# bruniss/multi-task-3d-resencoder-unet

Hardware: AMD Instinct MI355X
Metric: train patches/sec (b,c,z,y,x) ResEncM 1x128^3 (higher is better)
Workload: dtype bf16; 1 GPU; cfg2: ResEncM (6 stages, feats [32, 64, 128, 256, 512, 512], blocks [1, 3, 4, 6, 6, 6]), 1-in, heads ['sheet'], patch 128x128x128, batch 2/GPU, full train step (fwd+loss+bwd+allreduce+clip+AdamW); global_batch=2, parallelism=dp1

## Files before the change

include/rxunet.h:

```cpp
#ifndef RXUNET_H
#define RXUNET_H

#include <stddef.h>
#include <stdint.h>

#ifdef __cplusplus
extern "C" {
#endif

#define RX_OK 0
#define RX_EINVAL (-1)
#define RX_EUNSUPPORTED (-2)
#define RX_ELAUNCH (-3)
#define RX_EWORKSPACE (-4)

typedef enum { RX_F32 = 0, RX_BF16 = 1, RX_F16 = 2 } rx_dtype;
typedef enum { RX_ACT_NONE = 0, RX_ACT_SIGMOID = 1, RX_ACT_SOFTMAX = 2 } rx_head_act;

typedef struct {
  void* ptr;
  int32_t n, z, y, x, c, ld;
  int64_t cs;
} rx_act;

// ... 72 lines not shown
                   const float* gate, const float* mult, float* dadd, float* m12, float* dw1, float* db1, float* dw2,
                   float* db2, void* ws, size_t ws_bytes, void* stream);
int rx_instnorm_gate_act_bwd(rx_dtype dt, const rx_act* g, const rx_act* y, const float* stats, const rx_act* out,
                             float slope, const float* mult, const float* dadd, const float* m12, int keep_x,
                             const rx_act* dy, const rx_act* d_residual, int accumulate_residual, void* stream);

int rx_avgpool_fwd(rx_dtype dt, const rx_act* x, const rx_act* y, const int32_t stride[3], void* stream);
int rx_instnorm_act_pool_fwd(rx_dtype dt, const rx_act* y, const float* stats, const rx_act* residual,
                             const rx_act* out, const rx_act* pooled, const int32_t stride[3], float slope,
                             void* stream);
int rx_avgpool_bwd(rx_dtype dt, const rx_act* dy, const rx_act* dx, const int32_t stride[3], int accumulate,
                   void* stream);

int rx_stem_conv_fwd(rx_dtype dt, const float* x_ncdhw, int n, int cin, int z, int y, int x, const float* w,
                     const float* bias, const rx_act* out, const int32_t kernel[3], void* stream);
int rx_stem_conv_fwd_stats(rx_dtype dt, const float* x_ncdhw, int n, int cin, int z, int y, int x, const float* w,
                           const float* bias, const rx_act* out, const int32_t kernel[3], float eps, float* stats,
                           void* ws, size_t ws_bytes, void* stream);
size_t rx_stem_conv_bwd_weight_workspace(int cin, int cout, int taps);
int rx_stem_conv_bwd_weight(rx_dtype dt, const float* x_ncdhw, int n, int cin, int z, int y, int x,
                            const rx_act* dy, float* dw, const int32_t kernel[3], void* ws, size_t ws_bytes,
                            void* stream);

int rx_head_fwd(rx_dtype dt, const rx_act* x, const float* w, const float* b, int k, float* out_ncdhw,
                int act, void* stream);
size_t rx_head_bwd_workspace(const rx_act* x, int k);
int rx_head_bwd(rx_dtype dt, const float* dout_ncdhw, const rx_act* x, const float* w, int k, const rx_act* dx,
                float* dw, float* db, void* ws, size_t ws_bytes, void* stream);

int rx_instnorm_act_head_fwd(rx_dtype dt, const rx_act* y, const float* stats, const rx_act* out, float slope,
                             const float* head_w, const float* head_b, int k, float* out_ncdhw, int act, void* stream);

int rx_instnorm_act_bwd_head(rx_dtype dt, const float* dout_ncdhw, int k, const float* head_w, const rx_act* y,
                             const float* stats, float slope, const rx_act* dy, float* head_dw, float* head_db, void* ws,
                             size_t ws_bytes, void* stream);

size_t rx_channel_sum_workspace(const rx_act* x);
int rx_channel_sum(rx_dtype dt, const rx_act* x, float* out, void* ws, size_t ws_bytes, void* stream);

size_t rx_loss_workspace(int n, int c, long v);
int rx_bce_dice_loss_fwd(const float* logits, const float* target, int n, int c, long v, float alpha, float beta,
                         float smoothing, float eps, float* loss, float* coef, void* ws, size_t ws_bytes,
                         void* stream);
int rx_bce_dice_loss_bwd(const float* logits, const float* target, int n, int c, long v, float alpha, float beta,
                         float smoothing, const float* coef, const float* grad_loss, float* dlogits, void* stream);
int rx_masked_cosine_loss_fwd(const float* pred, const float* target, int n, int c, long v, float* loss, float* coef,
// ... 87 lines not shown
```

multi-task-3d-resencoder-unet_amd/csrc/rx_elementwise.hip:

```cpp
#include <stdarg.h>

#include <math.h>

#include "rx_common.h"
#include <cstdlib>

static thread_local char g_err[512] = "";
void rx_set_error(const char* fmt, ...) {
  va_list ap;
  va_start(ap, fmt);
  vsnprintf(g_err, sizeof(g_err), fmt, ap);
  va_end(ap);
}
extern "C" const char* rx_last_error(void) { return g_err; }
static thread_local const char* g_last_kernel = "";
static thread_local int g_note_seq_ = 0;
void rx_note_kernel(const char* name) { g_last_kernel = name; ++g_note_seq_; }
int rx_note_seq(void) { return g_note_seq_; }
extern "C" const char* rx_last_conv_kernel(void) { return g_last_kernel; }
extern "C" int rx_abi_version(void) { return 1; }
extern "C" int rx_device_arch_ok(void) {
  int dev = 0;
  if (hipGetDevice(&dev) != hipSuccess) return 0;
  hipDeviceProp_t p;
// ... 1808 lines not shown
  (void)TT;
  for (int i = threadIdx.x; i < 27 * Co; i += 256) {
    int t = i / Co, co = i - t * Co;
    float s = red[0][t][co] + red[1][t][co] + red[2][t][co] + red[3][t][co];
    partial[(((size_t)blockIdx.x * Cin + ci) * 27 + t) * Co + co] = s;
  }
}

__global__ __launch_bounds__(256) void stem_wgrad_finalize(const float* __restrict__ partial, int nch, int Cin, int ky, int kx, int TT, int Co,
                                                           float* __restrict__ dw) {
  const int lane = threadIdx.x & 63;
  const int i = blockIdx.x * 4 + (threadIdx.x >> 6);
  if (i >= Co * Cin * TT) return;
  int co = i / (Cin * TT), r = i - co * (Cin * TT), ci = r / TT, t = r - ci * TT;
  int a = t / (ky * kx), b = (t / kx) % ky, c = t % kx;
  int slot = a * 9 + b * 3 + c;
  double s = 0.0;
  for (int k = lane; k < nch; k += 64) s += (double)partial[(((size_t)k * Cin + ci) * 27 + slot) * Co + co];
  s = wave_sum_d(s);
  if (lane == 0) dw[i] = (float)s;
}

int rx_stem_wgrad_mfma_try(rx_dtype dt, const float* x, int n, int cin, int z, int y, int xx, const rx_act* dy, const int32_t kernel[3],
                           float* partial, int max_blocks, int* nblocks_out, hipStream_t st);
#define RX_STEM_CHUNKS 1024
extern "C" size_t rx_stem_conv_bwd_weight_workspace(int cin, int cout, int taps) {
  (void)taps;
  return (size_t)RX_STEM_CHUNKS * cin * 27 * cout * sizeof(float) + 256;
}

extern "C" int rx_stem_conv_bwd_weight(rx_dtype dt, const float* x_ncdhw, int n, int cin, int z, int y, int x, const rx_act* dy, float* dw,
                                       const int32_t kernel[3], void* ws, size_t ws_bytes, void* stream) {
  RX_RECORD(stream, [=, dy_ = RxActV(dy), kernel_ = RxI3V(kernel)](void* s) { return rx_stem_conv_bwd_weight(dt, x_ncdhw, n, cin, z, y, x, dy_.p(), dw, kernel_.v, ws, ws_bytes, s); });
  int rc;
  if ((rc = check_vec_channels(dy, dt, "rx_stem_conv_bwd_weight(dy)"))) return rc;
  if ((rc = check_kernel13(kernel, "rx_stem_conv_bwd_weight"))) return rc;
  if (!x_ncdhw || !dw || !ws || cin < 1 || cin > 16) RX_FAIL(RX_EUNSUPPORTED, "rx_stem_conv_bwd_weight: 1 <= Cin <= 16");
  const int Co = dy->c;
  if (Co > 64 || Co % 4 || 64 % (Co / 4)) RX_FAIL(RX_EUNSUPPORTED, "rx_stem_conv_bwd_weight: Cout must be 4,8,16,32 or 64 (got %d)", Co);
  if (dy->n != n || dy->z != z || dy->y != y || dy->x != x) RX_FAIL(RX_EINVAL, "rx_stem_conv_bwd_weight: geometry mismatch");
  if (ws_bytes < rx_stem_conv_bwd_weight_workspace(cin, Co, 27)) RX_FAIL(RX_EWORKSPACE, "rx_stem_conv_bwd_weight: workspace too small");
  hipStream_t st0 = (hipStream_t)stream;
  {
    int nb = 0;
    if (rx_stem_wgrad_mfma_try(dt, x_ncdhw, n, cin, z, y, x, dy, kernel, (float*)ws, RX_STEM_CHUNKS, &nb, st0) == 1) {
      const int TT0 = kernel[0] * kernel[1] * kernel[2];
      int tot0 = Co * cin * TT0;
      hipLaunchKernelGGL(stem_wgrad_finalize, dim3((tot0 + 3) / 4), dim3(256), 0, st0, (const float*)ws, nb, cin, kernel[1], kernel[2],
                         TT0, Co, dw);
      RX_CHECK_LAUNCH("rx_stem_conv_bwd_weight(mfma)");
      return RX_OK;
    }
  }
  const long NV = (long)n * z * y * x;
  const int VPB = 256 / (Co / 4);
  long chunk = (NV + RX_STEM_CHUNKS - 1) / RX_STEM_CHUNKS;
  chunk = (chunk + VPB - 1) / VPB * VPB;
  int nch = (int)((NV + chunk - 1) / chunk);
  const int TT = kernel[0] * kernel[1] * kernel[2];
  hipStream_t st = (hipStream_t)stream;
  RX_DISPATCH_DTYPE(dt, T, {
    hipLaunchKernelGGL((stem_wgrad_kernel<T>), dim3(nch, 1, cin), dim3(256), 0, st, x_ncdhw, cin, z, y, x, (const T*)dy->ptr, dy->ld,
                       rx_act_voxels(dy) * dy->ld, Co, kernel[0], kernel[1], kernel[2], n, (int)chunk, (float*)ws);
    int tot = Co * cin * TT;
    hipLaunchKernelGGL(stem_wgrad_finalize, dim3((tot + 3) / 4), dim3(256), 0, st, (const float*)ws, nch, cin, kernel[1], kernel[2], TT, Co,
                       dw);
  });
  RX_CHECK_LAUNCH("rx_stem_conv_bwd_weight");
  return RX_OK;
}

#define RX_PACK_PB 40
#ifndef RX_PACK_THREADS
#define RX_PACK_THREADS 1024
#endif

template <typename T>
__device__ __forceinline__ void pack_tile(const float* __restrict__ w, int A, int B, int TT, unsigned inv_tt, T* __restrict__ same,
                                          int flip_same, T* __restrict__ swp, int flip_swap, const int a0, const int b0) {
  extern __shared__ __attribute__((aligned(16))) unsigned char pack_smem[];
  T* L = reinterpret_cast<T*>(pack_smem);
  const int rowlen = 32 * TT;
  const bool full = a0 + 32 <= A && b0 + 32 <= B && sizeof(T) == 2 && (B & 7) == 0 && (A & 7) == 0;
  if (full && TT > 1 && (rowlen & 3) == 0 && ((size_t)B * TT & 3) == 0) {
    const int q4 = rowlen >> 2;
    for (int q = threadIdx.x; q < 32 * q4; q += RX_PACK_THREADS) {
      const int a = q / q4, c = q - a * q4;
      const f32x4 v = *reinterpret_cast<const f32x4*>(w + ((size_t)(a0 + a) * B + b0) * TT + 4 * c);
#pragma unroll
      for (int j = 0; j < 4; ++j) {
        const unsigned r = 4 * c + j;
// ... 524 lines not shown
```

multi-task-3d-resencoder-unet_amd/csrc/rx_stem_wgrad.hip:

```cpp
#include "rx_common.h"

typedef __attribute__((address_space(3))) s16x4 lds_s16x4_s;

template <typename T>
__device__ inline u32x4 pack8(const float (&f)[8]) {
  T v[8];
#pragma unroll
  for (int j = 0; j < 8; ++j) v[j] = Elem<T>::from_f(f[j]);
  return *reinterpret_cast<u32x4*>(v);
}

template <typename T, int NB>
__global__ __launch_bounds__(256) void stem_wgrad_mfma_kernel(const float* __restrict__ x, int Cin, int N, int Z, int Y, int X,
                                                              const T* __restrict__ dy, int ldy, long sy, int kz, int ky, int kx,
                                                              int tiles_per_block, float* __restrict__ partial) {
  constexpr int TZ = 4, TY = 4, TX = 16, HY = TY + 2, HX = TX + 2, HV = (TZ + 2) * HY * HX;
  constexpr int CO = NB * 32;
  __shared__ __attribute__((aligned(16))) T sG[256 * CO];
  __shared__ float sX[4][HV + 8];
  const int tid = threadIdx.x, lane = tid & 63, wave = tid >> 6;
  const int tz_n = (Z + TZ - 1) / TZ, ty_n = (Y + TY - 1) / TY, tx_n = (X + TX - 1) / TX;
  const int NT = N * tz_n * ty_n * tx_n;
  const int t_begin = blockIdx.x * tiles_per_block, t_end = min(NT, t_begin + tiles_per_block);
  const long V = (long)Z * Y * X;
  const int pz = (kz - 1) / 2, py = (ky - 1) / 2, px = (kx - 1) / 2;

  const int tap = lane & 31, h = lane >> 5;
  const int ta = tap / 9, tb = (tap / 3) % 3, tc = tap % 3;
  const bool tap_ok = tap < 27 && ta < kz && tb < ky && tc < kx;
  const int toff = tap_ok ? ((ta - pz) * HY + (tb - py)) * HX + (tc - px) : 0;
  const int g16 = lane >> 4, half = g16 & 1, ah = g16 >> 1, l15 = lane & 15, q4 = l15 >> 2, p4 = l15 & 3;

  f32x16 acc[4][NB];
#pragma unroll
  for (int c = 0; c < 4; ++c)
#pragma unroll
    for (int a = 0; a < NB; ++a)
#pragma unroll
      for (int r = 0; r < 16; ++r) acc[c][a][r] = 0.f;

  constexpr int GP = CO / 8;
  constexpr int XP = (HV + 255) / 256;
  u32x4 gq[GP];
  float xq[4][XP];
  auto prefetch = [&](int tile) {
    int tx = tile % tx_n, t1 = tile / tx_n;
    int ty = t1 % ty_n, t2 = t1 / ty_n;
    int tz = t2 % tz_n, n = t2 / tz_n;
    const int z0 = tz * TZ, y0 = ty * TY, x0 = tx * TX;
#pragma unroll
    for (int p = 0; p < GP; ++p) {
      const int i = tid + 256 * p;
      const int v = i / (CO / 8), cv = i - v * (CO / 8);
      const int z = z0 + (v >> 6), y = y0 + ((v >> 4) & 3), xx = x0 + (v & 15);
      u32x4 val = u32x4{0u, 0u, 0u, 0u};
      if (z < Z && y < Y && xx < X) val = *reinterpret_cast<const u32x4*>(dy + n * sy + ((long)(z * Y + y) * X + xx) * ldy + cv * 8);
      gq[p] = val;
    }
#pragma unroll
    for (int ci = 0; ci < 4; ++ci) {
      if (ci < Cin) {
        const float* xc = x + ((long)n * Cin + ci) * V;
#pragma unroll
        for (int p = 0; p < XP; ++p) {
          const int i = tid + 256 * p;
          const int hx = i % HX, t = i / HX, hy = t % HY, hz = t / HY;
          const int z = z0 + hz - 1, y = y0 + hy - 1, xx = x0 + hx - 1;
          float v = 0.f;
          if (i < HV && (unsigned)z < (unsigned)Z && (unsigned)y < (unsigned)Y && (unsigned)xx < (unsigned)X) v = xc[((long)z * Y + y) * X + xx];
          xq[ci][p] = v;
        }
      }
    }
  };
  if (t_begin < t_end) prefetch(t_begin);
  for (int tile = t_begin; tile < t_end; ++tile) {
    __syncthreads();
#pragma unroll
    for (int p = 0; p < GP; ++p) {
      const int i = tid + 256 * p;
      const int v = i / (CO / 8), c = (i - v * (CO / 8)) * 8;
      *reinterpret_cast<u32x4*>(sG + ((c >> 5) * 256 + v) * 32 + (c & 31)) = gq[p];
    }
#pragma unroll
    for (int ci = 0; ci < 4; ++ci)
      if (ci < Cin)
#pragma unroll
        for (int p = 0; p < XP; ++p)
          if (tid + 256 * p < HV) sX[ci][tid + 256 * p] = xq[ci][p];
    __syncthreads();
    if (tile + 1 < t_end) prefetch(tile + 1);
#pragma unroll
    for (int kk = 0; kk < 4; ++kk) {
      const int s = wave * 4 + kk;
      const int hrow = (((s >> 2) + 1) * HY + ((s & 3) + 1)) * HX + 1;
      u32x4 af[NB];
#pragma unroll
      for (int a = 0; a < NB; ++a) {
        const T* p0 = sG + (a * 256 + 16 * s + 8 * ah + q4) * 32 + 16 * half + 4 * p4;
        s16x4 t0 = __builtin_amdgcn_ds_read_tr16_b64_v4i16((lds_s16x4_s*)(p0));
        s16x4 t1 = __builtin_amdgcn_ds_read_tr16_b64_v4i16((lds_s16x4_s*)(p0 + 4 * 32));
        u32x2 lo = __builtin_bit_cast(u32x2, t0), hi = __builtin_bit_cast(u32x2, t1);
        af[a] = u32x4{lo[0], lo[1], hi[0], hi[1]};
      }
      for (int ci = 0; ci < Cin; ++ci) {
// ... 13 lines not shown
    }
  }
  __shared__ float red[4][32][33];
  const int col = lane & 31, fh = lane >> 5;
  for (int ci = 0; ci < Cin; ++ci)
    for (int a = 0; a < NB; ++a) {
      __syncthreads();
#pragma unroll
      for (int r = 0; r < 16; ++r) {
        const int row = (r & 3) + 8 * (r >> 2) + 4 * fh;
        float v = ci == 0 ? acc[0][a][r] : ci == 1 ? acc[1][a][r] : ci == 2 ? acc[2][a][r] : acc[3][a][r];
        red[wave][row][col] = v;
      }
      __syncthreads();
      for (int i = tid; i < 27 * 32; i += 256) {
        const int t = i >> 5, co = i & 31;
        float s = red[0][co][t] + red[1][co][t] + red[2][co][t] + red[3][co][t];
        partial[(((size_t)blockIdx.x * Cin + ci) * 27 + t) * CO + a * 32 + co] = s;
      }
    }
}

int rx_stem_wgrad_mfma_try(rx_dtype dt, const float* x, int n, int cin, int z, int y, int xx, const rx_act* dy, const int32_t kernel[3],
                           float* partial, int max_blocks, int* nblocks_out, hipStream_t st) {
  if (dt == RX_F32 || (dy->c != 32 && dy->c != 64) || dy->ld % 8 || ((uintptr_t)dy->ptr & 15) || cin > 4) return 0;
  const int NT = n * ((z + 3) / 4) * ((y + 3) / 4) * ((xx + 15) / 16);
  int blocks = NT < max_blocks ? NT : max_blocks;
  if (blocks > 768) blocks = 768;
  const int per = (NT + blocks - 1) / blocks;
  blocks = (NT + per - 1) / per;
  const long sy = rx_act_voxels(dy) * (long)dy->ld;
#define RX_SW(TT, NBB)                                                                                                           \
  hipLaunchKernelGGL((stem_wgrad_mfma_kernel<TT, NBB>), dim3(blocks), dim3(256), 0, st, x, cin, n, z, y, xx, (const TT*)dy->ptr, \
                     dy->ld, sy, kernel[0], kernel[1], kernel[2], per, partial)
  if (dt == RX_BF16) {
    if (dy->c == 32) RX_SW(bf16_t, 1); else RX_SW(bf16_t, 2);
  } else {
    if (dy->c == 32) RX_SW(f16_t, 1); else RX_SW(f16_t, 2);
  }
#undef RX_SW
  *nblocks_out = blocks;
  return 1;
}


#define RX_STEM_NOTAP 0x40000000
template <typename T, bool STATS = false, int KSM = 7>
__global__ __launch_bounds__(256) void stem_fwd_mfma_kernel(const float* __restrict__ x, int Cin, int N, int Z, int Y, int X,
                                                            const float* __restrict__ w, const float* __restrict__ bias, T* __restrict__ out,
                                                            int ldo, long so, int kz, int ky, int kx, int tiles_per_block,
                                                            int blocks_per_sample = 0, float* __restrict__ stat_part = nullptr) {
  constexpr int TZ = 4, TY = 4, TX = 16, HY = TY + 2, HX = TX + 2, HV = (TZ + 2) * HY * HX;
  constexpr int XP = (HV + 255) / 256;
  __shared__ float sX[4][HV + 8];
  __shared__ int sOff[128];
  const int tid = threadIdx.x, lane = tid & 63, wave = tid >> 6;
  const int TT = kz * ky * kx, K = Cin * TT, KS = (K + 15) / 16;
// ... 155 lines not shown
```

multi-task-3d-resencoder-unet_amd/engine/lib.py:

```python
import ctypes
import os
from ctypes import POINTER, c_char_p, c_double, c_float, c_int, c_int32, c_long, c_size_t, c_void_p

import torch

_HERE = os.path.dirname(os.path.abspath(__file__))
LIB_PATH = os.environ.get("RX_LIBRARY") or os.path.join(os.path.dirname(_HERE), "csrc", "librxunet.so")

RX_F32, RX_BF16, RX_F16 = 0, 1, 2
RX_ACT_NONE, RX_ACT_SIGMOID, RX_ACT_SOFTMAX = 0, 1, 2
DTYPE_CODE = {torch.float32: RX_F32, torch.bfloat16: RX_BF16, torch.float16: RX_F16}
RX_SW_U8, RX_SW_U16, RX_SW_F32 = 0, 1, 2
RX_SW_SCALE, RX_SW_ZSCORE = 0, 1
RX_SW_BLEND_AVERAGE, RX_SW_BLEND_UNIT, RX_SW_BLEND_NONE = 0, 1, 2
RX_SW_CAST_U8, RX_SW_CAST_U16 = 0, 1
RX_AUG_PW_NONE, RX_AUG_PW_AFFINE, RX_AUG_PW_PLANE, RX_AUG_PW_NOISE = 0, 1, 2, 3
RX_AUG_G3_NONE, RX_AUG_G3_FILTER, RX_AUG_G3_DOWNSCALE = 0, 1, 2
RX_AUG_MAX_K, RX_AUG_MAX_BOXES = 21, 4


class RxError(RuntimeError):
    pass


# ... 38 lines not shown
    "rx_instnorm_stats_mask": (c_int, [c_void_p, c_void_p, c_int, c_void_p]),
    "rx_instnorm_fwd": (c_int, [c_int, _P, c_float, c_void_p, _P, _P, c_float, c_void_p, c_size_t, c_void_p]),
    "rx_instnorm_act_bwd": (c_int, [c_int, _P, _P, c_void_p, _P, c_float, _P, _P, c_int, c_void_p, c_size_t,
                                    c_void_p]),
    "rx_instnorm_act_bwd_res": (c_int, [c_int, _P, _P, c_void_p, _P, c_float, _P, I3, _P, _P, c_void_p, c_size_t, c_void_p]),
    "rx_se_workspace": (c_size_t, [_P]),
    "rx_se_gate_fwd": (c_int, [c_int, _P, c_void_p, c_void_p, _PSE, c_void_p, c_void_p, c_void_p, c_void_p, c_void_p, c_size_t,
                               c_void_p]),
    "rx_instnorm_gate_act_fwd": (c_int, [c_int, _P, c_void_p, c_void_p, c_int, _P, _P, c_float, c_void_p]),
    "rx_se_gate_bwd": (c_int, [c_int, _P, _P, c_void_p, _P, c_float, c_void_p, _PSE, c_void_p, c_void_p, c_void_p, c_void_p,
                               c_void_p, c_void_p, c_void_p, c_void_p, c_void_p, c_void_p, c_void_p, c_size_t, c_void_p]),
    "rx_instnorm_gate_act_bwd": (c_int, [c_int, _P, _P, c_void_p, _P, c_float, c_void_p, c_void_p, c_void_p, c_int, _P, _P,
                                         c_int, c_void_p]),
    "rx_avgpool_fwd": (c_int, [c_int, _P, _P, I3, c_void_p]),
    "rx_instnorm_act_pool_fwd": (c_int, [c_int, _P, c_void_p, _P, _P, _P, I3, c_float, c_void_p]),
    "rx_avgpool_bwd": (c_int, [c_int, _P, _P, I3, c_int, c_void_p]),
    "rx_stem_conv_fwd": (c_int, [c_int, c_void_p, c_int, c_int, c_int, c_int, c_int, c_void_p, c_void_p, _P, I3,
                                 c_void_p]),
    "rx_stem_conv_fwd_stats": (c_int, [c_int, c_void_p, c_int, c_int, c_int, c_int, c_int, c_void_p, c_void_p, _P, I3,
                                       c_float, c_void_p, c_void_p, c_size_t, c_void_p]),
    "rx_stem_conv_bwd_weight_workspace": (c_size_t, [c_int, c_int, c_int]),
    "rx_stem_conv_bwd_weight": (c_int, [c_int, c_void_p, c_int, c_int, c_int, c_int, c_int, _P, c_void_p, I3,
                                        c_void_p, c_size_t, c_void_p]),
    "rx_head_fwd": (c_int, [c_int, _P, c_void_p, c_void_p, c_int, c_void_p, c_int, c_void_p]),
    "rx_head_bwd_workspace": (c_size_t, [_P, c_int]),
    "rx_instnorm_act_head_fwd": (c_int, [c_int, _P, c_void_p, _P, c_float, c_void_p, c_void_p, c_int, c_void_p, c_int, c_void_p]),
    "rx_instnorm_act_bwd_head": (c_int, [c_int, c_void_p, c_int, c_void_p, _P, c_void_p, c_float, _P, c_void_p, c_void_p, c_void_p, c_size_t,
                                         c_void_p]),
    "rx_grad_norm_clip_partials": (ctypes.c_long, [c_int, c_void_p]),
    "rx_grad_norm_clip": (c_int, [c_int, c_void_p, c_void_p, c_float, c_void_p, ctypes.c_long, c_void_p, c_void_p]),
    "rx_head_bwd": (c_int, [c_int, c_void_p, _P, c_void_p, c_int, _P, c_void_p, c_void_p, c_void_p, c_size_t,
                            c_void_p]),
    "rx_channel_sum_workspace": (c_size_t, [_P]),
    "rx_channel_sum": (c_int, [c_int, _P, c_void_p, c_void_p, c_size_t, c_void_p]),
    "rx_loss_workspace": (c_size_t, [c_int, c_int, c_long]),
    "rx_bce_dice_loss_fwd": (c_int, [c_void_p, c_void_p, c_int, c_int, c_long, c_float, c_float, c_float, c_float, c_void_p,
                                     c_void_p, c_void_p, c_size_t, c_void_p]),
    "rx_bce_dice_loss_bwd": (c_int, [c_void_p, c_void_p, c_int, c_int, c_long, c_float, c_float, c_float, c_void_p, c_void_p,
                                     c_void_p, c_void_p]),
    "rx_masked_cosine_loss_fwd": (c_int, [c_void_p, c_void_p, c_int, c_int, c_long, c_void_p, c_void_p, c_void_p, c_size_t,
                                          c_void_p]),
    "rx_masked_cosine_loss_bwd": (c_int, [c_void_p, c_void_p, c_int, c_int, c_long, c_void_p, c_void_p, c_void_p, c_void_p]),
    "rx_adamw_pack": (c_int, [c_int, c_void_p, c_void_p, c_void_p, c_void_p, c_void_p, c_double, c_double, c_double, c_double, c_double,
                              c_int, c_int, c_int, c_int, c_int, c_void_p, c_void_p, c_void_p]),
    "rx_adamw_flat_multi": (c_int, [c_int, c_void_p, c_void_p, c_void_p, c_void_p, c_void_p, c_void_p, c_double, c_double, c_double,
                                    c_double, c_double, c_int, c_void_p]),
# ... 80 lines not shown
```

multi-task-3d-resencoder-unet_amd/engine/ops.py:

```python
from ctypes import byref, c_void_p

import numpy as np
import torch

from . import lib as _l
from .lib import I3, RxAct, check, load, stream_ptr

_WS = {}
_PROF = None


def set_profiler(p):
    global _PROF
    _PROF = p


class LaunchProfiler:

    def __init__(self):
        self.pending = []
        self.groups = {}
        self.pending_hbm = []
        self.hbm = {}

# ... 450 lines not shown

def stem_conv_fwd(x_ncdhw, w, bias, out, kernel):
    n, cin, z, y, x = x_ncdhw.shape
    assert x_ncdhw.dtype == torch.float32 and x_ncdhw.is_contiguous()
    check(load().rx_stem_conv_fwd(_code(out.dtype), _ptr(x_ncdhw), n, cin, z, y, x, _ptr(w), _ptr(bias),
                                  byref(out.desc()), I3(*kernel), stream_ptr()), "rx_stem_conv_fwd")


def stem_conv_fwd_stats(x_ncdhw, w, bias, out, kernel, stats, eps=1e-5, ws=None):
    n, cin, z, y, x = x_ncdhw.shape
    assert x_ncdhw.dtype == torch.float32 and x_ncdhw.is_contiguous()
    ws = workspace() if ws is None else ws
    check(load().rx_stem_conv_fwd_stats(_code(out.dtype), _ptr(x_ncdhw), n, cin, z, y, x, _ptr(w), _ptr(bias),
                                        byref(out.desc()), I3(*kernel), float(eps), _ptr(stats), *_ws_args(ws), stream_ptr()),
          "rx_stem_conv_fwd_stats")


def stem_conv_bwd_weight(x_ncdhw, dy, dw, kernel, ws=None):
    n, cin, z, y, x = x_ncdhw.shape
    need = load().rx_stem_conv_bwd_weight_workspace(cin, dy.c, 27)
    ws = workspace(need) if ws is None else ws
    check(load().rx_stem_conv_bwd_weight(_code(dy.dtype), _ptr(x_ncdhw), n, cin, z, y, x, byref(dy.desc()), _ptr(dw),
                                         I3(*kernel), *_ws_args(ws), stream_ptr()), "rx_stem_conv_bwd_weight")


def head_fwd(x, w, b, out_ncdhw, act=_l.RX_ACT_NONE):
    k = w.shape[0]
    check(load().rx_head_fwd(_code(x.dtype), byref(x.desc()), _ptr(w), _ptr(b), k, _ptr(out_ncdhw), int(act),
                             stream_ptr()), "rx_head_fwd")


def head_bwd(dout_ncdhw, x, w, dx, dw, db, ws=None):
    k = w.shape[0]
    need = load().rx_head_bwd_workspace(byref(x.desc()), k)
    ws = workspace(need) if ws is None else ws
    check(load().rx_head_bwd(_code(x.dtype), _ptr(dout_ncdhw), byref(x.desc()), _ptr(w), k,
                             byref(dx.desc()) if dx is not None else None, _ptr(dw), _ptr(db), *_ws_args(ws),
                             stream_ptr()), "rx_head_bwd")


def instnorm_act_head_fwd(y, stats, out, w, b, out_ncdhw, act, slope=0.01):
    check(load().rx_instnorm_act_head_fwd(_code(y.dtype), byref(y.desc()), _ptr(stats), byref(out.desc()) if out is not None else None,
                                          float(slope), _ptr(w), _ptr(b), w.shape[0], _ptr(out_ncdhw), int(act), stream_ptr()),
          "rx_instnorm_act_head_fwd")


# ... 153 lines not shown
se_gate_fwd = _hbm("se_gate_fwd(linesum+gate)", lambda y, *a, **k: _tb(y))(se_gate_fwd)
instnorm_gate_act_fwd = _hbm("in_gate_act_fwd", lambda y, stats, mult, keep_x, out, slope=0.01, residual=None:
                             _tb(y) + _tb(out) + _tb(residual))(instnorm_gate_act_fwd)
se_gate_bwd = _hbm("se_gate_bwd(linesums+gate)", lambda g, y, stats, out, *a, **k: _tb(g) + _tb(y) + _tb(out))(se_gate_bwd)
instnorm_gate_act_bwd = _hbm("in_gate_act_bwd",
                             lambda g, y, stats, out, slope, mult, dadd, m12, keep_x, dy, d_residual=None, accumulate_residual=False:
                             _bwd_bytes(g, y, out, dy, d_residual, accumulate_residual))(instnorm_gate_act_bwd)
avgpool_fwd = _hbm("avgpool_fwd", lambda x, y, stride: _tb(x) + _tb(y))(avgpool_fwd)
instnorm_act_pool_fwd = _hbm("in_act_pool_fwd", lambda y, stats, out, pooled, stride, slope=0.01, residual=None:
                             _tb(y) + _tb(out) + _tb(pooled) + _tb(residual))(instnorm_act_pool_fwd)
avgpool_bwd = _hbm("avgpool_bwd", lambda dy, dx, stride, accumulate=False: _tb(dy) + _tb(dx) * (2 if accumulate else 1))(avgpool_bwd)
head_fwd = _hbm("head_fwd", lambda x, w, b, out_ncdhw, act=0: _tb(x) + out_ncdhw.numel() * 4)(head_fwd)
head_bwd = _hbm("head_bwd", lambda dout_ncdhw, x, w, dx, dw, db, ws=None: dout_ncdhw.numel() * 4 + _tb(x) + _tb(dx))(head_bwd)
instnorm_act_head_fwd = _hbm("in_act_head_fwd", lambda y, stats, out, w, b, out_ncdhw, act, slope=0.01:
                             _tb(y) + _tb(out) + out_ncdhw.numel() * 4)(instnorm_act_head_fwd)
instnorm_act_bwd_head = _hbm("in_act_bwd_head(colreduce+apply)", lambda dout_ncdhw, w, y, stats, dy, slope=0.01, ws=None, dw=None, db=None:
                             dout_ncdhw.numel() * 4 + _tb(y) + _tb(dy))(instnorm_act_bwd_head)
channel_sum = _hbm("channel_sum", lambda x, out, ws=None: _tb(x))(channel_sum)
pack_conv_weight = _hbm("pack", _pack_bytes)(pack_conv_weight)
pack_convT_weight = _hbm("pack", _pack_bytes)(pack_convT_weight)
stem_conv_fwd = _hbm("stem_conv_fwd", lambda x_ncdhw, w, bias, out, kernel: x_ncdhw.numel() * 4 + _tb(out))(stem_conv_fwd)
stem_conv_fwd_stats = _hbm("stem_conv_fwd", lambda x_ncdhw, w, bias, out, kernel, stats, eps=1e-5, ws=None: x_ncdhw.numel() * 4 + _tb(out))(stem_conv_fwd_stats)
stem_conv_bwd_weight = _hbm("stem_conv_bwd_weight", lambda x_ncdhw, dy, dw, kernel, ws=None: x_ncdhw.numel() * 4 + _tb(dy))(stem_conv_bwd_weight)
convT3d_fwd = _hbm("convT_fwd", lambda x, w_fwd, bias, y, stride, ws=None: _tb(x) + _tb(y))(convT3d_fwd)
convT3d_bwd_data = _hbm("convT_bwd_data", lambda dy, w_bwd, dx, stride, accumulate=False, ws=None:
                        _tb(dy) + _tb(dx) * (2 if accumulate else 1))(convT3d_bwd_data)
convT3d_bwd_weight = _hbm("convT_bwd_weight", lambda x, dy, dw, stride, ws=None: _tb(x) + _tb(dy))(convT3d_bwd_weight)
```

multi-task-3d-resencoder-unet_amd/engine/plan.py:

```python
from dataclasses import dataclass, field
from typing import Callable, Dict, List, Optional

import os

import torch
from torch import nn

from . import lib as _l
from . import ops
from .ops import Act


class UnsupportedConfig(NotImplementedError):
    pass


_SIDE_STREAMS: Dict[str, "torch.cuda.Stream"] = {}


def side_stream(device):
    key = str(device)
    st = _SIDE_STREAMS.get(key)
    if st is None:
        st = _SIDE_STREAMS[key] = torch.cuda.Stream(device=device)
# ... 57 lines not shown
        spatial = tuple(in_shape[2:])
        if self.two_d:
            spatial = (1,) + spatial
        self.B, self.Cin, self.spatial = B, Cin, spatial

        self.params: List[nn.Parameter] = []
        self._pidx: Dict[int, int] = {}
        self.packs: List[dict] = []
        self.enc_tape: List[Rec] = []
        self.dec_tapes: List[List[Rec]] = []
        self.fwd: List[Callable] = []
        self.bwd: List[Callable] = []
        self.dy_pool: Dict[tuple, Act] = {}
        self._gbase: Dict[int, torch.Tensor] = {}
        self.outputs: Dict[str, torch.Tensor] = {}
        self.bytes_alloc = 0
        self._x = None
        self._dlogits: Dict[str, torch.Tensor] = {}
        self._grads: List[Optional[torch.Tensor]] = []
        self.grad_order: List[int] = []
        self.grad_sync = None
        import os
        self.overlap_wgrad = os.environ.get("RX_OVERLAP_WGRAD", "1") != "0"
        self.dy_ring = 4
        self._side = None
        self._ws2 = None
        self._dy_turn: Dict[tuple, int] = {}
        self._dy_free: Dict[int, int] = {}
        self._dy_ev: Dict[int, int] = {}
        self._ev_fork = None
        self._ev_join = None
        self._pack_groups = None
        self._gates: List[dict] = []
        self._drops: List[dict] = []
        self._shadows: List[dict] = []
        self._shadow_of: Dict[int, dict] = {}
        self._pad_idx: Dict[int, dict] = {}
        self._pad_done: List[int] = []
        self.use_programs = os.environ.get("RX_PROGRAMS", "1") == "1"
        self._pstate: Dict[tuple, dict] = {}
        self._gflat = None
        self._gviews: Dict[int, torch.Tensor] = {}
        self._marks: List[tuple] = []
        self._recording = None
        self._on_side = False
        self._use_gstore = False
# ... 512 lines not shown
                        f.append(lambda a=a: ops.avgpool_fwd(a["x"].act, a["y"].act, a["stride"]))
                elif rec.kind == "copy":
                    f.append(lambda a=a: ops.avgpool_fwd(a["x"].act, a["y"].act, (1, 1, 1)))
                elif rec.kind == "head":
                    if a.get("fwd_fused"):
                        continue

                    def step(a=a):
                        w2 = a["w"].view(a["k"], -1)
                        ops.head_fwd(a["x"].act, w2, a["b"], a["out"], a["act"] if P._apply_act else _l.RX_ACT_NONE)
                    f.append(step)

    def _dy_for(self, y: AT):
        key = (y.act.dims, y.act.c)
        turn = self._dy_turn.get(key, 0)
        self._dy_turn[key] = (turn + 1) % self.dy_ring
        slot = key + (turn,)
        if slot not in self.dy_pool:
            t = torch.empty((*y.act.dims, y.act.c), dtype=self.dtype, device=self.device)
            self.bytes_alloc += t.numel() * t.element_size()
            self.dy_pool[slot] = Act(t)
        return self.dy_pool[slot]

    def _gen_backward(self):
        P = self
        b = self.bwd
        cat_written = {}

        def mark_cat(cat):
            cat_written[cat.act.key] = True

        def view_written(at):
            return at.written or cat_written.get(at.act.key, False)

        def new_grad(idx):
            sync = P.grad_sync
            ent = P._pad_idx.get(idx)
            if ent is not None:
                if ent["gpad"] is None:
                    ent["gpad"] = torch.empty(tuple(ent["sh"].shape), dtype=torch.float32, device=P.device)
                P._pad_done.append(idx)
                return ent["gpad"]
            if sync is not None:
                g = sync.alloc(idx)
            elif P._use_gstore:
                g = P._gviews[idx]
# ... 60 lines not shown

                    def step(a=a, gx=gx, hinfo=hinfo):
                        dl = P._dlogits.get(a["name"])
                        if dl is None:
                            gx.t.zero_()
                            if P.grad_sync is not None:
                                for i in (a["widx"], a["bidx"]):
                                    new_grad(i).zero_()
                                    done(i)
                            return
                        if hinfo.get("dw_fused"):
                            return
                        dw, db = new_grad(a["widx"]), new_grad(a["bidx"])
                        ops.head_bwd(dl, a["x"].act, a["w"].view(a["k"], -1), None if hinfo["fused"] else gx, dw, db)
                        done(a["widx"])
                        done(a["bidx"])
                    order += [a["widx"], a["bidx"]]
                    b.append(step)
                elif rec.kind == "inact":
                    out, y, res = a["out"], a["y"], a["res"]
                    gout = self._grad_buf(out) if out.gact is None else out.gact
                    if not view_written(out):
                        raise RuntimeError(f"plan bug: gradient of {out.name} is consumed before it is produced")
                    dy = self._dy_for(y)
                    y.gact = dy
                    gres, acc = None, False
                    if res is not None and res.needs_grad:
                        gres = self._grad_buf(res)
                        acc = view_written(res)
                        res.written = True
                        wrote(res, "gres")
                    gw = getattr(out, "_gw", (None, None))
                    if (gw[0] == "head" and a["gate"] is None and res is None and self.dtype != torch.float32
                            and out.act.voxels > 512):
                        heads = [r.a for r in tape if r.kind == "head" and r.a["x"] is out]
                        if len(heads) == 1 and heads[0]["k"] <= 4:
                            a["head_src"] = heads[0]
                            gw[1]["fused"] = True
                            if heads[0].get("fwd_fused") and heads[0]["w"] is self.params[heads[0]["widx"]]:
                                a["head_dw_fused"] = True
                                gw[1]["dw_fused"] = True
                    if (gw[0] == "conv" and a["gate"] is None and res is None and self.dtype != torch.float32
                            and out.act.full_buffer and out.act.root is None and out.act.c % 32 == 0 and out.act.voxels > 512
                            and out.act.dims[3] >= 16):
                        a["m12"] = torch.empty((self.B, out.act.c, 2), dtype=torch.float32, device=self.device)
                        a["m12_valid"] = False
                        gw[1]["inact"] = a
                    def gistep(a=a, gout=gout, dy=dy, gres=gres, acc=acc):
                        g = a["gate"]
                        before_dy_write(dy)
                        if g["se"] is None and g.get("scale_now") is None:
                            ops.instnorm_act_bwd(gout, a["y"].act, a["stats"],
                                                 a["out"].act if (a["slope"] != 1.0 and a["res"] is not None) else None, dy,
                                                 a["slope"], gres, acc)
                            return
                        grads = [new_grad(i) for i in g["se"]["idx"]] if g["se"] is not None else [None] * 4
                        ops.se_gate_bwd(gout, a["y"].act, a["stats"], a["out"].act, a["slope"], P._se_args(g), g["pooled"],
                                        g["hidden"], g["gate"], g["mult"], g["dadd"], g["m12"], *grads,
                                        path_scale=g.get("scale_now"))
                        ops.instnorm_gate_act_bwd(gout, a["y"].act, a["stats"], a["out"].act, a["slope"], g["mult"], g["dadd"],
                                                  g["m12"], g["keep_x"], dy, gres, acc)
                        if g["se"] is not None:
                            for i in g["se"]["idx"]:
                                done(i)
                    if a["gate"] is not None:
                        if a["gate"]["se"] is not None:
                            order += a["gate"]["se"]["idx"]
                        b.append(gistep)
                        continue

                    pend = getattr(out, "_pool_pending", None)
                    out._pool_pending = None
                    fuse_res = gres is not None and not acc and res is not None and y.act.voxels > 512
                    if pend is not None and not fuse_res:
                        b.append(lambda pend=pend: ops.avgpool_bwd(pend["gy"], pend["gx"], pend["stride"], True))
                        pend = None
                    if fuse_res:
                        def rstep(a=a, gout=gout, dy=dy, gres=gres, pend=pend):
                            before_dy_write(dy)
                            ops.instnorm_act_bwd_res(gout, a["y"].act, a["stats"], a["out"].act, dy, gres, a["slope"],
                                                     pool_dy=pend["gy"] if pend is not None else None,
                                                     pool_stride=pend["stride"] if pend is not None else (1, 1, 1))
                        b.append(rstep)
                        continue

                    def istep(a=a, gout=gout, dy=dy, gres=gres, acc=acc):
                        before_dy_write(dy)
                        mask_out = a["out"].act if (a["slope"] != 1.0 and a["res"] is not None) else None
                        hs = a.get("head_src")
                        dl = P._dlogits.get(hs["name"]) if hs is not None else None
                        if dl is not None and a.get("head_dw_fused"):
                            dw, db = new_grad(hs["widx"]), new_grad(hs["bidx"])
                            ops.instnorm_act_bwd_head(dl, hs["w"].view(hs["k"], -1), a["y"].act, a["stats"], dy, a["slope"],
                                                      dw=dw.view(hs["k"], -1), db=db)
                            done(hs["widx"])
                            done(hs["bidx"])
                        elif dl is not None:
                            ops.instnorm_act_bwd_head(dl, hs["w"].view(hs["k"], -1), a["y"].act, a["stats"], dy, a["slope"])
                        elif a.get("m12_valid"):
                            a["m12_valid"] = False
                            ops.instnorm_act_bwd_apply(gout, a["y"].act, a["stats"], mask_out, dy, a["m12"], a["slope"], gres, acc)
                        elif "inbwd_reduce" in skip and a["y"].act.voxels > 512:
                            if "m12x" not in a:
                                a["m12x"] = torch.zeros((self.B, a["y"].act.c, 2), dtype=torch.float32, device=self.device)
                            ops.instnorm_act_bwd_apply(gout, a["y"].act, a["stats"], mask_out, dy, a["m12x"], a["slope"], gres, acc)
                        else:
                            ops.instnorm_act_bwd(gout, a["y"].act, a["stats"], mask_out, dy, a["slope"], gres, acc)
                    b.append(istep)
                elif rec.kind in ("conv", "stem"):
                    y = a["y"]
                    dy = y.gact

                    def wstep(a=a, dy=dy, kind=rec.kind):
                        dw = new_grad(a["widx"])
                        db = new_grad(a["bidx"]) if a["bidx"] is not None else None

                        def launches(ws):
                            if "wgrad" in skip and kind != "stem":
                                pass
                            elif kind == "stem":
                                ops.stem_conv_bwd_weight(P._x, dy, dw, a["kernel"], ws)
                            else:
                                ops.conv3d_bwd_weight(a["x"].act, dy, dw, a["kernel"], a["stride"], ws)
                            done(a["widx"])
                            if db is not None:
                                ops.channel_sum(dy, db, ws)
                                done(a["bidx"])
                        side_run(launches, dy)
                    order += [a["widx"]] + ([a["bidx"]] if a["bidx"] is not None else [])
                    b.append(wstep)
                    if rec.kind == "conv" and a["x"].needs_grad:
                        x = a["x"]
                        gx = self._grad_buf(x)
                        acc = view_written(x)
                        x.written = True
                        if x.act.full_buffer:
                            mark_cat(x)
# ... 439 lines not shown
            if g is None:
                continue
            g = g.detach()
            if g.dtype != torch.float32 or not g.is_contiguous():
                g = g.float().contiguous()
            if graphs or programs:
                buf = self._dl_static.get(k)
                if buf is None or buf.shape != g.shape:
                    buf = self._dl_static[k] = torch.empty_like(g)
                buf.copy_(g)
                g = buf
            self._dlogits[k] = g.unsqueeze(2) if self.two_d else g
        self._ensure_side()
        self.net._weights_epoch = getattr(self.net, "_weights_epoch", 0) + 1
        self._grads = [None] * len(self.params)
        if programs:
            sync = self.grad_sync
            self._use_gstore = sync is None
            if sync is None:
                self._grad_store()
            else:
                sync.persistent = True
                sync.begin(self)
            key = ("b", tuple(sorted(self._dlogits)), id(sync) if sync is not None else 0, self.overlap_wgrad)
            st, replayed = self._programmed(key, self._backward_body,
                                            segments=self._replay_backward_segments if sync is not None else None)
            if replayed:
                self._pad_done = [idx for idx in set(self.grad_order) if idx in self._pad_idx]
            if replayed and sync is None:
                for idx in set(self.grad_order):
                    self._grads[idx] = self._gviews[idx]
            grads = self._backward_finish()
            return [t.detach() if t is not None else None for t in grads]
        self._use_gstore = False
        if self.grad_sync is not None:
            self.grad_sync.persistent = False
            self.grad_sync.begin(self)
        if not graphs:
            self._backward_body()
            return self._backward_finish()
        key = ("b", tuple(sorted(self._dlogits)))
        st = self._gstate.get(key)
        if st is not None and st.get("graph") is not None:
            owned = st["owned"]
            for p in self.params:
                gr = p.grad
                if gr is not None and gr.data_ptr() in owned:
                    p.grad = gr.clone()

        def body():
            self._backward_body()
            return self._backward_finish()
        st = self._graphed(key, body)
        grads = st["result"]
        if st["eager"]:
            return grads
        if "owned" not in st:
            st["owned"] = {t.data_ptr() for t in grads if t is not None}
        return [t.detach() if t is not None else None for t in grads]
```

Before: 119.4 patches/s.

## Fuse instnorm-activation backward into stem conv weight-gradient kernel

Adds an INACT variant of the stem MFMA wgrad kernel. It recomputes the instance-norm plus leaky-ReLU backward (dy from g, y, stats, m12) on the fly while staging tiles into shared memory. The planner detects the stem conv followed by an instnorm whose residual needs no gradient, and skips materialising the full-resolution stem dy tensor and the separate wgrad read of it. In exchange the kernel does extra loads of y and per-channel stats. There is also a fallback path that allocates a dy buffer lazily when fusion is not applicable.

Result: no change. 119.7 patches/s, median of 4 (+0.3%).

```diff
diff --git a/include/rxunet.h b/include/rxunet.h
--- a/include/rxunet.h
+++ b/include/rxunet.h
@@ -118,6 +118,10 @@
                             const rx_act* dy, float* dw, const int32_t kernel[3], void* ws, size_t ws_bytes,
                             void* stream);
 
+int rx_stem_conv_bwd_weight_inact(rx_dtype dt, const float* x_ncdhw, int n, int cin, int z, int y, int x, const rx_act* g,
+                                  const rx_act* in_y, const float* in_stats, const float* m12, float slope, float* dw,
+                                  const int32_t kernel[3], int* fused, void* ws, size_t ws_bytes, void* stream);
+
 int rx_head_fwd(rx_dtype dt, const rx_act* x, const float* w, const float* b, int k, float* out_ncdhw,
                 int act, void* stream);
 size_t rx_head_bwd_workspace(const rx_act* x, int k);
diff --git a/multi-task-3d-resencoder-unet_amd/csrc/rx_elementwise.hip b/multi-task-3d-resencoder-unet_amd/csrc/rx_elementwise.hip
--- a/multi-task-3d-resencoder-unet_amd/csrc/rx_elementwise.hip
+++ b/multi-task-3d-resencoder-unet_amd/csrc/rx_elementwise.hip
@@ -1854,7 +1854,8 @@
 }
 
 int rx_stem_wgrad_mfma_try(rx_dtype dt, const float* x, int n, int cin, int z, int y, int xx, const rx_act* dy, const int32_t kernel[3],
-                           float* partial, int max_blocks, int* nblocks_out, hipStream_t st);
+                           float* partial, int max_blocks, int* nblocks_out, hipStream_t st, const rx_act* in_y,
+                           const float* in_stats, const float* m12, float slope);
 #define RX_STEM_CHUNKS 1024
 extern "C" size_t rx_stem_conv_bwd_weight_workspace(int cin, int cout, int taps) {
   (void)taps;
@@ -1875,7 +1876,8 @@
   hipStream_t st0 = (hipStream_t)stream;
   {
     int nb = 0;
-    if (rx_stem_wgrad_mfma_try(dt, x_ncdhw, n, cin, z, y, x, dy, kernel, (float*)ws, RX_STEM_CHUNKS, &nb, st0) == 1) {
+    if (rx_stem_wgrad_mfma_try(dt, x_ncdhw, n, cin, z, y, x, dy, kernel, (float*)ws, RX_STEM_CHUNKS, &nb, st0, nullptr, nullptr, nullptr,
+                               1.f) == 1) {
       const int TT0 = kernel[0] * kernel[1] * kernel[2];
       int tot0 = Co * cin * TT0;
       hipLaunchKernelGGL(stem_wgrad_finalize, dim3((tot0 + 3) / 4), dim3(256), 0, st0, (const float*)ws, nb, cin, kernel[1], kernel[2],
@@ -1899,6 +1901,34 @@
                        dw);
   });
   RX_CHECK_LAUNCH("rx_stem_conv_bwd_weight");
+  return RX_OK;
+}
+
+extern "C" int rx_stem_conv_bwd_weight_inact(rx_dtype dt, const float* x_ncdhw, int n, int cin, int z, int y, int x, const rx_act* g,
+                                             const rx_act* in_y, const float* in_stats, const float* m12, float slope, float* dw,
+                                             const int32_t kernel[3], int* fused, void* ws, size_t ws_bytes, void* stream) {
+  RX_RECORD(stream, [=, g_ = RxActV(g), in_y_ = RxActV(in_y), kernel_ = RxI3V(kernel)](void* s) { int fused_dummy = 0; return rx_stem_conv_bwd_weight_inact(dt, x_ncdhw, n, cin, z, y, x, g_.p(), in_y_.p(), in_stats, m12, slope, dw, kernel_.v, &fused_dummy, ws, ws_bytes, s); });
+  if (!fused) RX_FAIL(RX_EINVAL, "rx_stem_conv_bwd_weight_inact: bad arguments");
+  *fused = 0;
+  int rc;
+  if ((rc = check_vec_channels(g, dt, "rx_stem_conv_bwd_weight_inact(g)"))) return rc;
+  if ((rc = check_vec_channels(in_y, dt, "rx_stem_conv_bwd_weight_inact(in_y)"))) return rc;
+  if ((rc = check_kernel13(kernel, "rx_stem_conv_bwd_weight_inact"))) return rc;
+  if (!x_ncdhw || !dw || !ws || !in_stats || cin < 1 || cin > 16) RX_FAIL(RX_EINVAL, "rx_stem_conv_bwd_weight_inact: bad arguments");
+  if (!same_geom(in_y, g) || g->n != n || g->z != z || g->y != y || g->x != x)
+    RX_FAIL(RX_EINVAL, "rx_stem_conv_bwd_weight_inact: geometry mismatch");
+  const int Co = g->c;
+  if (dt == RX_F32 || (Co != 32 && Co != 64) || cin > 4 || !m12) return RX_OK;
+  if (ws_bytes < rx_stem_conv_bwd_weight_workspace(cin, Co, 27)) RX_FAIL(RX_EWORKSPACE, "rx_stem_conv_bwd_weight_inact: workspace too small");
+  hipStream_t st = (hipStream_t)stream;
+  int nb = 0;
+  if (rx_stem_wgrad_mfma_try(dt, x_ncdhw, n, cin, z, y, x, g, kernel, (float*)ws, RX_STEM_CHUNKS, &nb, st, in_y, in_stats, m12, slope) != 1)
+    return RX_OK;
+  const int TT = kernel[0] * kernel[1] * kernel[2];
+  hipLaunchKernelGGL(stem_wgrad_finalize, dim3((Co * cin * TT + 3) / 4), dim3(256), 0, st, (const float*)ws, nb, cin, kernel[1], kernel[2], TT,
+                     Co, dw);
+  RX_CHECK_LAUNCH("rx_stem_conv_bwd_weight_inact");
+  *fused = 1;
   return RX_OK;
 }
 
diff --git a/multi-task-3d-resencoder-unet_amd/csrc/rx_stem_wgrad.hip b/multi-task-3d-resencoder-unet_amd/csrc/rx_stem_wgrad.hip
--- a/multi-task-3d-resencoder-unet_amd/csrc/rx_stem_wgrad.hip
+++ b/multi-task-3d-resencoder-unet_amd/csrc/rx_stem_wgrad.hip
@@ -10,10 +10,13 @@
   return *reinterpret_cast<u32x4*>(v);
 }
 
-template <typename T, int NB>
+template <typename T, int NB, bool INACT = false>
 __global__ __launch_bounds__(256) void stem_wgrad_mfma_kernel(const float* __restrict__ x, int Cin, int N, int Z, int Y, int X,
                                                               const T* __restrict__ dy, int ldy, long sy, int kz, int ky, int kx,
-                                                              int tiles_per_block, float* __restrict__ partial) {
+                                                              int tiles_per_block, float* __restrict__ partial,
+                                                              const T* __restrict__ yc = nullptr, int ldc = 0, long sc = 0,
+                                                              const float* __restrict__ stats = nullptr,
+                                                              const float* __restrict__ m12 = nullptr, float slope = 1.f) {
   constexpr int TZ = 4, TY = 4, TX = 16, HY = TY + 2, HX = TX + 2, HV = (TZ + 2) * HY * HX;
   constexpr int CO = NB * 32;
   __shared__ __attribute__((aligned(16))) T sG[256 * CO];
@@ -42,7 +45,11 @@
   constexpr int GP = CO / 8;
   constexpr int XP = (HV + 255) / 256;
   u32x4 gq[GP];
+  u32x4 yq[INACT ? GP : 1];
+  unsigned gok = 0;
   float xq[4][XP];
+  float cmean[INACT ? 8 : 1], crstd[INACT ? 8 : 1], cm1[INACT ? 8 : 1], cm2[INACT ? 8 : 1];
+  int cn = -1;
   auto prefetch = [&](int tile) {
     int tx = tile % tx_n, t1 = tile / tx_n;
     int ty = t1 % ty_n, t2 = t1 / ty_n;
@@ -54,8 +61,15 @@
       const int v = i / (CO / 8), cv = i - v * (CO / 8);
       const int z = z0 + (v >> 6), y = y0 + ((v >> 4) & 3), xx = x0 + (v & 15);
       u32x4 val = u32x4{0u, 0u, 0u, 0u};
-      if (z < Z && y < Y && xx < X) val = *reinterpret_cast<const u32x4*>(dy + n * sy + ((long)(z * Y + y) * X + xx) * ldy + cv * 8);
+      const bool in = z < Z && y < Y && xx < X;
+      if (in) val = *reinterpret_cast<const u32x4*>(dy + n * sy + ((long)(z * Y + y) * X + xx) * ldy + cv * 8);
       gq[p] = val;
+      if (INACT) {
+        u32x4 yv = u32x4{0u, 0u, 0u, 0u};
+        if (in) yv = *reinterpret_cast<const u32x4*>(yc + n * sc + ((long)(z * Y + y) * X + xx) * ldc + cv * 8);
+        yq[p] = yv;
+        gok = in ? gok | (1u << p) : gok & ~(1u << p);
+      }
     }
 #pragma unroll
     for (int ci = 0; ci < 4; ++ci) {
@@ -76,11 +90,39 @@
   if (t_begin < t_end) prefetch(t_begin);
   for (int tile = t_begin; tile < t_end; ++tile) {
     __syncthreads();
+    if (INACT) {
+      const int n = tile / (tz_n * ty_n * tx_n);
+      if (n != cn) {
+        cn = n;
+#pragma unroll
+        for (int j = 0; j < 8; ++j) {
+          const size_t k = (size_t)n * CO + (tid % (CO / 8)) * 8 + j;
+          cmean[j] = stats[2 * k];
+          crstd[j] = stats[2 * k + 1];
+          cm1[j] = m12[2 * k];
+          cm2[j] = m12[2 * k + 1];
+        }
+      }
+    }
 #pragma unroll
     for (int p = 0; p < GP; ++p) {
       const int i = tid + 256 * p;
       const int v = i / (CO / 8), c = (i - v * (CO / 8)) * 8;
-      *reinterpret_cast<u32x4*>(sG + ((c >> 5) * 256 + v) * 32 + (c & 31)) = gq[p];
+      u32x4 val = gq[p];
+      if (INACT) {
+        T gv[8], yv[8], dv[8];
+        *reinterpret_cast<u32x4*>(gv) = gq[p];
+        *reinterpret_cast<u32x4*>(yv) = yq[p];
+#pragma unroll
+        for (int j = 0; j < 8; ++j) {
+          float gg = Elem<T>::to_f(gv[j]);
+          float xh = (Elem<T>::to_f(yv[j]) - cmean[j]) * crstd[j];
+          if (slope != 1.0f && !(xh > 0.f)) gg *= slope;
+          dv[j] = Elem<T>::from_f(crstd[j] * (gg - cm1[j] - xh * cm2[j]));
+        }
+        val = (gok >> p) & 1u ? *reinterpret_cast<u32x4*>(dv) : u32x4{0u, 0u, 0u, 0u};
+      }
+      *reinterpret_cast<u32x4*>(sG + ((c >> 5) * 256 + v) * 32 + (c & 31)) = val;
     }
 #pragma unroll
     for (int ci = 0; ci < 4; ++ci)
@@ -140,17 +182,27 @@
 }
 
 int rx_stem_wgrad_mfma_try(rx_dtype dt, const float* x, int n, int cin, int z, int y, int xx, const rx_act* dy, const int32_t kernel[3],
-                           float* partial, int max_blocks, int* nblocks_out, hipStream_t st) {
+                           float* partial, int max_blocks, int* nblocks_out, hipStream_t st, const rx_act* in_y,
+                           const float* in_stats, const float* m12, float slope) {
   if (dt == RX_F32 || (dy->c != 32 && dy->c != 64) || dy->ld % 8 || ((uintptr_t)dy->ptr & 15) || cin > 4) return 0;
+  if (in_y && (in_y->c != dy->c || in_y->ld % 8 || ((uintptr_t)in_y->ptr & 15) || !in_stats || !m12)) return 0;
   const int NT = n * ((z + 3) / 4) * ((y + 3) / 4) * ((xx + 15) / 16);
   int blocks = NT < max_blocks ? NT : max_blocks;
   if (blocks > 768) blocks = 768;
   const int per = (NT + blocks - 1) / blocks;
   blocks = (NT + per - 1) / per;
   const long sy = rx_act_voxels(dy) * (long)dy->ld;
-#define RX_SW(TT, NBB)                                                                                                           \
-  hipLaunchKernelGGL((stem_wgrad_mfma_kernel<TT, NBB>), dim3(blocks), dim3(256), 0, st, x, cin, n, z, y, xx, (const TT*)dy->ptr, \
-                     dy->ld, sy, kernel[0], kernel[1], kernel[2], per, partial)
+#define RX_SW(TT, NBB)                                                                                                             \
+  do {                                                                                                                             \
+    if (in_y)                                                                                                                      \
+      hipLaunchKernelGGL((stem_wgrad_mfma_kernel<TT, NBB, true>), dim3(blocks), dim3(256), 0, st, x, cin, n, z, y, xx,             \
+                         (const TT*)dy->ptr, dy->ld, sy, kernel[0], kernel[1], kernel[2], per, partial, (const TT*)in_y->ptr,      \
+                         in_y->ld, rx_act_voxels(in_y) * (long)in_y->ld, in_stats, m12, slope);                                    \
+    else                                                                                                                           \
+      hipLaunchKernelGGL((stem_wgrad_mfma_kernel<TT, NBB, false>), dim3(blocks), dim3(256), 0, st, x, cin, n, z, y, xx,            \
+                         (const TT*)dy->ptr, dy->ld, sy, kernel[0], kernel[1], kernel[2], per, partial, (const TT*)nullptr, 0, 0L, \
+                         (const float*)nullptr, (const float*)nullptr, 1.f);                                                       \
+  } while (0)
   if (dt == RX_BF16) {
     if (dy->c == 32) RX_SW(bf16_t, 1); else RX_SW(bf16_t, 2);
   } else {
diff --git a/multi-task-3d-resencoder-unet_amd/engine/lib.py b/multi-task-3d-resencoder-unet_amd/engine/lib.py
--- a/multi-task-3d-resencoder-unet_amd/engine/lib.py
+++ b/multi-task-3d-resencoder-unet_amd/engine/lib.py
@@ -84,6 +84,8 @@
     "rx_stem_conv_bwd_weight_workspace": (c_size_t, [c_int, c_int, c_int]),
     "rx_stem_conv_bwd_weight": (c_int, [c_int, c_void_p, c_int, c_int, c_int, c_int, c_int, _P, c_void_p, I3,
                                         c_void_p, c_size_t, c_void_p]),
+    "rx_stem_conv_bwd_weight_inact": (c_int, [c_int, c_void_p, c_int, c_int, c_int, c_int, c_int, _P, _P, c_void_p, c_void_p, c_float,
+                                              c_void_p, I3, POINTER(c_int), c_void_p, c_size_t, c_void_p]),
     "rx_head_fwd": (c_int, [c_int, _P, c_void_p, c_void_p, c_int, c_void_p, c_int, c_void_p]),
     "rx_head_bwd_workspace": (c_size_t, [_P, c_int]),
     "rx_instnorm_act_head_fwd": (c_int, [c_int, _P, c_void_p, _P, c_float, c_void_p, c_void_p, c_int, c_void_p, c_int, c_void_p]),
diff --git a/multi-task-3d-resencoder-unet_amd/engine/ops.py b/multi-task-3d-resencoder-unet_amd/engine/ops.py
--- a/multi-task-3d-resencoder-unet_amd/engine/ops.py
+++ b/multi-task-3d-resencoder-unet_amd/engine/ops.py
@@ -496,6 +496,18 @@
     ws = workspace(need) if ws is None else ws
     check(load().rx_stem_conv_bwd_weight(_code(dy.dtype), _ptr(x_ncdhw), n, cin, z, y, x, byref(dy.desc()), _ptr(dw),
                                          I3(*kernel), *_ws_args(ws), stream_ptr()), "rx_stem_conv_bwd_weight")
+
+
+def stem_conv_bwd_weight_inact(x_ncdhw, g, in_y, in_stats, m12, slope, dw, kernel, ws=None):
+    from ctypes import c_int
+    n, cin, z, y, x = x_ncdhw.shape
+    need = load().rx_stem_conv_bwd_weight_workspace(cin, g.c, 27)
+    ws = workspace(need) if ws is None else ws
+    fused = c_int(0)
+    check(load().rx_stem_conv_bwd_weight_inact(_code(g.dtype), _ptr(x_ncdhw), n, cin, z, y, x, byref(g.desc()), byref(in_y.desc()),
+                                               _ptr(in_stats), _ptr(m12), float(slope), _ptr(dw), I3(*kernel), byref(fused),
+                                               *_ws_args(ws), stream_ptr()), "rx_stem_conv_bwd_weight_inact")
+    return bool(fused.value)
 
 
 def head_fwd(x, w, b, out_ncdhw, act=_l.RX_ACT_NONE):
@@ -695,6 +707,8 @@
 stem_conv_fwd = _hbm("stem_conv_fwd", lambda x_ncdhw, w, bias, out, kernel: x_ncdhw.numel() * 4 + _tb(out))(stem_conv_fwd)
 stem_conv_fwd_stats = _hbm("stem_conv_fwd", lambda x_ncdhw, w, bias, out, kernel, stats, eps=1e-5, ws=None: x_ncdhw.numel() * 4 + _tb(out))(stem_conv_fwd_stats)
 stem_conv_bwd_weight = _hbm("stem_conv_bwd_weight", lambda x_ncdhw, dy, dw, kernel, ws=None: x_ncdhw.numel() * 4 + _tb(dy))(stem_conv_bwd_weight)
+stem_conv_bwd_weight_inact = _hbm("stem_conv_bwd_weight_inact", lambda x_ncdhw, g, in_y, in_stats, m12, slope, dw, kernel, ws=None:
+                                  x_ncdhw.numel() * 4 + _tb(g) + _tb(in_y))(stem_conv_bwd_weight_inact)
 convT3d_fwd = _hbm("convT_fwd", lambda x, w_fwd, bias, y, stride, ws=None: _tb(x) + _tb(y))(convT3d_fwd)
 convT3d_bwd_data = _hbm("convT_bwd_data", lambda dy, w_bwd, dx, stride, accumulate=False, ws=None:
                         _tb(dy) + _tb(dx) * (2 if accumulate else 1))(convT3d_bwd_data)
diff --git a/multi-task-3d-resencoder-unet_amd/engine/plan.py b/multi-task-3d-resencoder-unet_amd/engine/plan.py
--- a/multi-task-3d-resencoder-unet_amd/engine/plan.py
+++ b/multi-task-3d-resencoder-unet_amd/engine/plan.py
@@ -103,6 +103,7 @@
         self.grad_sync = None
         import os
         self.overlap_wgrad = os.environ.get("RX_OVERLAP_WGRAD", "1") != "0"
+        self.fuse_stem_bwd = True
         self.dy_ring = 4
         self._side = None
         self._ws2 = None
@@ -661,6 +662,14 @@
             self.dy_pool[slot] = Act(t)
         return self.dy_pool[slot]
 
+    def _stem_dy(self, a):
+        if "dy" not in a:
+            y = a["y"].act
+            t = torch.empty((*y.dims, y.c), dtype=self.dtype, device=self.device)
+            self.bytes_alloc += t.numel() * t.element_size()
+            a["dy"] = Act(t)
+        return a["dy"]
+
     def _gen_backward(self):
         P = self
         b = self.bwd
@@ -767,8 +776,6 @@
                     gout = self._grad_buf(out) if out.gact is None else out.gact
                     if not view_written(out):
                         raise RuntimeError(f"plan bug: gradient of {out.name} is consumed before it is produced")
-                    dy = self._dy_for(y)
-                    y.gact = dy
                     gres, acc = None, False
                     if res is not None and res.needs_grad:
                         gres = self._grad_buf(res)
@@ -791,6 +798,16 @@
                         a["m12"] = torch.empty((self.B, out.act.c, 2), dtype=torch.float32, device=self.device)
                         a["m12_valid"] = False
                         gw[1]["inact"] = a
+                    ti = next(i for i, r in enumerate(tape) if r is rec)
+                    prev = tape[ti - 1] if ti > 0 else None
+                    if ("m12" in a and gres is None and prev is not None and prev.kind == "stem" and prev.a["y"] is y
+                            and prev.a["bidx"] is None and self.Cin <= 4 and y.act.c in (32, 64)):
+                        a["stem_fuse"] = prev.a
+                        prev.a["dy_from"] = a
+                        dy = None
+                    else:
+                        dy = self._dy_for(y)
+                    y.gact = dy
                     def gistep(a=a, gout=gout, dy=dy, gres=gres, acc=acc):
                         g = a["gate"]
                         before_dy_write(dy)
@@ -830,6 +847,18 @@
                         continue
 
                     def istep(a=a, gout=gout, dy=dy, gres=gres, acc=acc):
+                        sf = a.get("stem_fuse")
+                        if sf is not None:
+                            if P.fuse_stem_bwd and a.get("m12_valid"):
+                                dw = new_grad(sf["widx"])
+                                if ops.stem_conv_bwd_weight_inact(P._x, gout, a["y"].act, a["stats"], a["m12"], a["slope"], dw,
+                                                                  sf["kernel"]):
+                                    a["m12_valid"] = False
+                                    done(sf["widx"])
+                                    sf["dw_fused"] = True
+                                    return
+                                sf["dw_pre"] = dw
+                            dy = P._stem_dy(a)
                         before_dy_write(dy)
                         mask_out = a["out"].act if (a["slope"] != 1.0 and a["res"] is not None) else None
                         hs = a.get("head_src")
@@ -857,7 +886,13 @@
                     dy = y.gact
 
                     def wstep(a=a, dy=dy, kind=rec.kind):
-                        dw = new_grad(a["widx"])
+                        if a.pop("dw_fused", False):
+                            return
+                        if dy is None:
+                            dy = P._stem_dy(a["dy_from"])
+                        dw = a.pop("dw_pre", None)
+                        if dw is None:
+                            dw = new_grad(a["widx"])
                         db = new_grad(a["bidx"]) if a["bidx"] is not None else None
 
                         def launches(ws):
@@ -1343,7 +1378,7 @@
             else:
                 sync.persistent = True
                 sync.begin(self)
-            key = ("b", tuple(sorted(self._dlogits)), id(sync) if sync is not None else 0, self.overlap_wgrad)
+            key = ("b", tuple(sorted(self._dlogits)), id(sync) if sync is not None else 0, self.overlap_wgrad, self.fuse_stem_bwd)
             st, replayed = self._programmed(key, self._backward_body,
                                             segments=self._replay_backward_segments if sync is not None else None)
             if replayed:
@@ -1360,7 +1395,7 @@
         if not graphs:
             self._backward_body()
             return self._backward_finish()
-        key = ("b", tuple(sorted(self._dlogits)))
+        key = ("b", tuple(sorted(self._dlogits)), self.fuse_stem_bwd)
         st = self._gstate.get(key)
         if st is not None and st.get("graph") is not None:
             owned = st["owned"]
```
